# Kainmueller-Lab/PatchPerPix

Hardware: AMD Instinct MI355X
Metric: Mvoxels/sec assembled (vote_instances) (higher is better)
Workload: dtype f16 in, f32 accumulate

## Files before the change

### include/ppp_mi355x.h

```cpp
#ifndef PPP_MI355X_H
#define PPP_MI355X_H

#include <stddef.h>
#include <stdint.h>

#ifdef __cplusplus
extern "C" {
#endif

#define PPP_ABI_VERSION 5

enum ppp_error {
    PPP_OK = 0,
    PPP_ERR_INVALID_ARG = -1,
    PPP_ERR_NO_DEVICE = -2,
    PPP_ERR_HIP = -3,
    PPP_ERR_UNSUPPORTED = -4,
    PPP_ERR_WORKSPACE = -5
};

enum ppp_dtype { PPP_F32 = 0, PPP_F16 = 1, PPP_BF16 = 2 };

enum ppp_bg_rule { PPP_BG_INV_TH = 0, PPP_BG_HALF_TH = 1, PPP_BG_LESS_THAN_TH = 2 };
enum ppp_value_rule { PPP_VAL_COUNT = 0, PPP_VAL_PROB_PRODUCT = 1, PPP_VAL_NORM_PROB_PRODUCT = 2 };
// ... 50 lines not shown

int64_t ppp_consensus_sparse_workspace_bytes(const ppp_params *p, const ppp_box *part);
int ppp_consensus_sparse(const void *d_pred, int pred_dtype, const uint8_t *d_overlap, float *d_cons,
                         float *d_count, const ppp_params *p, const ppp_box *part, int open_rows, void *d_work,
                         int mode, void *stream);
void ppp_consensus_last_items(int64_t *total, int64_t *active, int *took_lists);

int ppp_rank_patches(const void *d_pred, int pred_dtype, const float *d_cons,
                     const uint8_t *d_overlap, float *d_score, const ppp_box *score_box,
                     const ppp_params *p, void *stream);

int64_t ppp_rank_workspace_bytes(const ppp_box *score_box, const ppp_params *p);
int ppp_rank_patches_vm(const void *d_pred, int pred_dtype, const float *d_cons_vm,
                        const uint8_t *d_overlap, float *d_score, const ppp_box *score_box,
                        void *d_work, const ppp_params *p, void *stream);

int ppp_patch_graph(const void *d_pred, int pred_dtype, const float *d_cons,
                    const uint32_t *d_pairs, const uint32_t *d_order, uint64_t n_pairs,
                    float *d_aff, const ppp_params *p, void *stream);

int32_t ppp_patch_graph_by_patch_chunk(const ppp_params *p);
int32_t ppp_patch_graph_by_patch_chunk_small(const ppp_params *p);
int ppp_patch_graph_by_patch_chunked(const void *d_pred, int pred_dtype, const float *d_cons_vm,
                                     const uint32_t *d_pairs, const uint32_t *d_order,
                                     const int64_t *d_group_start, const int64_t *d_chunk_offsets,
                                     int32_t n_groups, int64_t n_blocks, int32_t chunk, float *d_aff,
                                     const ppp_params *p, void *stream);
int64_t ppp_patch_graph_lcg_words(int32_t dz, int32_t dy, int32_t dx, const ppp_params *p);
int ppp_patch_graph_lcg(const void *d_pred, int pred_dtype, const uint32_t *d_pairs,
                        const uint32_t *d_order, const int64_t *d_lcg_pos, int64_t n_lcg,
// ... 291 lines not shown
```

### patchperpix_amd/backend.py

```python
import ctypes
import os

import numpy as np

from . import build as _build

F32, F16, BF16 = 0, 1, 2
BG_INV_TH, BG_HALF_TH, BG_LESS_THAN_TH = 0, 1, 2
VAL_COUNT, VAL_PROB_PRODUCT, VAL_NORM_PROB_PRODUCT = 0, 1, 2
CONS_COMPACT, CONS_REFERENCE, CONS_VOXEL_MAJOR = 0, 1, 2
ABI_VERSION = 5
NONE_KEY = 0xFFFFFFFF
NONE_KEY64 = 1 << 62
PAIR_KEY_FAR = 0x7FFFFFFFFFFFFFFF


class Box(ctypes.Structure):
    _fields_ = [(n, ctypes.c_int32) for n in ("z0", "y0", "x0", "z1", "y1", "x1")]

    def shape(self):
        return (self.z1 - self.z0, self.y1 - self.y0, self.x1 - self.x0)


class Params(ctypes.Structure):
# ... 66 lines not shown
                                          ctypes.c_void_p, ctypes.POINTER(Params), ctypes.POINTER(Box),
                                          ctypes.c_void_p]),
    "ppp_consensus_sparse_workspace_bytes": (ctypes.c_int64, [ctypes.POINTER(Params), ctypes.POINTER(Box)]),
    "ppp_consensus_sparse": (ctypes.c_int, [ctypes.c_void_p, ctypes.c_int, ctypes.c_void_p, ctypes.c_void_p,
                                            ctypes.c_void_p, ctypes.POINTER(Params), ctypes.POINTER(Box),
                                            ctypes.c_int, ctypes.c_void_p, ctypes.c_int, ctypes.c_void_p]),
    "ppp_consensus_last_items": (None, [ctypes.POINTER(ctypes.c_int64), ctypes.POINTER(ctypes.c_int64),
                                        ctypes.POINTER(ctypes.c_int)]),
    "ppp_cons_planes_to_rows": (ctypes.c_int, [ctypes.c_void_p, ctypes.POINTER(Box), ctypes.c_void_p,
                                               ctypes.POINTER(Params), ctypes.c_void_p]),
    "ppp_rank_patches": (ctypes.c_int, [ctypes.c_void_p, ctypes.c_int, ctypes.c_void_p,
                                        ctypes.c_void_p, ctypes.c_void_p,
                                        ctypes.POINTER(Box), ctypes.POINTER(Params),
                                        ctypes.c_void_p]),
    "ppp_rank_workspace_bytes": (ctypes.c_int64, [ctypes.POINTER(Box), ctypes.POINTER(Params)]),
    "ppp_rank_patches_vm": (ctypes.c_int, [ctypes.c_void_p, ctypes.c_int, ctypes.c_void_p,
                                           ctypes.c_void_p, ctypes.c_void_p, ctypes.POINTER(Box),
                                           ctypes.c_void_p, ctypes.POINTER(Params), ctypes.c_void_p]),
    "ppp_patch_graph": (ctypes.c_int, [ctypes.c_void_p, ctypes.c_int, ctypes.c_void_p,
                                       ctypes.c_void_p, ctypes.c_void_p, ctypes.c_uint64,
                                       ctypes.c_void_p, ctypes.POINTER(Params),
                                       ctypes.c_void_p]),
    "ppp_patch_graph_by_patch": (ctypes.c_int, [ctypes.c_void_p, ctypes.c_int, ctypes.c_void_p,
                                                ctypes.c_void_p, ctypes.c_void_p, ctypes.c_void_p,
                                                ctypes.c_void_p, ctypes.c_int32, ctypes.c_int64,
                                                ctypes.c_void_p, ctypes.POINTER(Params),
                                                ctypes.c_void_p]),
    "ppp_patch_graph_by_patch_chunk_small": (ctypes.c_int32, [ctypes.POINTER(Params)]),
    "ppp_patch_graph_by_patch_chunked": (ctypes.c_int, [ctypes.c_void_p, ctypes.c_int, ctypes.c_void_p,
                                                        ctypes.c_void_p, ctypes.c_void_p, ctypes.c_void_p,
# ... 681 lines not shown
        lo3 = [max(sb[a] - rad[a], (cb.z0, cb.y0, cb.x0)[a]) for a in range(3)]
        hi3 = [min(sb[3 + a] + rad[a], (cb.z1, cb.y1, cb.x1)[a]) for a in range(3)]
        note_add("s2_base_voxels", int(np.prod([max(0, h - l) for l, h in zip(lo3, hi3)])))
        with _timed("rank_patches"):
            check(lib().ppp_rank_patches_vm(_dev_ptr(pred), pred_dtype_code(pred), _dev_ptr(cons),
                                            _dev_ptr(overlap), _dev_ptr(out), box, _dev_ptr(work),
                                            ctypes.byref(P), _stream()))
        return out
    with _timed("rank_patches"):
        check(lib().ppp_rank_patches(_dev_ptr(pred), pred_dtype_code(pred), _dev_ptr(cons),
                                     _dev_ptr(overlap), _dev_ptr(out), box, ctypes.byref(P),
                                     _stream()))
    return out


def rank_vm_available(P):
    if os.environ.get("PPP_RANK", "vm") != "vm":
        return False
    Pv = P.copy()
    Pv.cons_layout = CONS_VOXEL_MAJOR
    Pv.cons_box = Box(0, 0, 0, P.Z, P.Y, P.X)
    if P.ring_z and P.ring_z < P.Z:
        Pv.cons_box = Box(0, 0, 0, P.ring_z, P.Y, P.X)
        sb = Box(0, 0, 0, max(1, P.ring_z - P.pz // 2), P.Y, P.X)
        return int(lib().ppp_rank_workspace_bytes(ctypes.byref(sb), ctypes.byref(Pv))) > 0
    return int(lib().ppp_rank_workspace_bytes(None, ctypes.byref(Pv))) > 0


def pair_order(pairs, P):
    torch = _torch()
# ... 1163 lines not shown
```

### patchperpix_amd/csrc/ppp_api.hip

```cpp
#include <cmath>
#include <cstdarg>
#include <cstdio>
#include <cstring>

#include "ppp_kernels.hpp"

namespace {

thread_local char g_err[512] = "";

int fail(int code, const char *fmt, ...) {
    va_list ap;
    va_start(ap, fmt);
    vsnprintf(g_err, sizeof(g_err), fmt, ap);
    va_end(ap);
    return code;
}

int hip_fail(hipError_t e, const char *what) {
    return fail(PPP_ERR_HIP, "%s: %s", what, hipGetErrorString(e));
}

float round_down_f32(double t) {
    float f = (float)t;
// ... 283 lines not shown
    if (!ppp::cons_box_covers(G, *sb))
        return fail(PPP_ERR_INVALID_ARG, "cons_box does not cover score_box grown by the patch radius");
    return PPP_OK;
}

int64_t ppp_rank_workspace_bytes(const ppp_box *score_box, const ppp_params *p) {
    ppp::Geo G;
    if (make_geo(p, &G) != PPP_OK) return -1;
    if (!ppp::rank_vm_supported(G)) return 0;
    if (G.ring && !ppp::rank_wg_supported(G)) return 0;
    ppp_box sb;
    if (rank_box(score_box, p, G, &sb) != PPP_OK) return -1;
    return (int64_t)ppp::rank_vm_workspace_bytes(sb, G);
}

#ifdef PPP_RW_STAMPS
extern "C" int64_t ppp_rank_wg_stamps_offset(const ppp_box *score_box, const ppp_params *p) {
    ppp::Geo G;
    ppp_box sb;
    if (make_geo(p, &G) != PPP_OK || !ppp::rank_wg_supported(G) || rank_box(score_box, p, G, &sb) != PPP_OK) return -1;
    return (int64_t)ppp::rank_wg_stamps_offset(sb, G);
}
#endif

int ppp_rank_patches_vm(const void *d_pred, int pred_dtype, const float *d_cons_vm,
                        const uint8_t *d_overlap, float *d_score, const ppp_box *score_box,
                        void *d_work, const ppp_params *p, void *stream) {
    ppp::Geo G;
    PPP_TRY(make_geo(p, &G));
    PPP_TRY(check_dtype(pred_dtype));
// ... 1259 lines not shown
```

### patchperpix_amd/csrc/ppp_kernels.hpp

```cpp
#pragma once
#include <stdlib.h>
#include <string.h>
#include "ppp_common.hpp"

namespace ppp {

int env_epoch();
void env_reload();
struct EnvSwitch {
    const char *name;
    int seen = -1;
    bool is_set = false;
    char val[32] = {0};
    explicit EnvSwitch(const char *n) : name(n) {}
    const char *get() {
        if (seen != env_epoch()) {
            const char *e = getenv(name);
            is_set = e != nullptr;
            if (e) { strncpy(val, e, sizeof(val) - 1); val[sizeof(val) - 1] = 0; }
            seen = env_epoch();
        }
        return is_set ? val : nullptr;
    }
};
// ... 27 lines not shown
hipError_t launch_consensus_part(const void *pred, int dtype, const uint8_t *ov, float *cons, const Geo &G,
                                 hipStream_t s);
bool consensus_v4_supported(const Geo &G);
hipError_t launch_consensus_v4(const void *pred, int dtype, const uint8_t *ov, float *cons,
                               float *cnt, const Geo &G, hipStream_t s);
hipError_t launch_rank(const void *pred, int dtype, const float *cons, const uint8_t *ov,
                       float *score, const ppp_box &sb, const Geo &G, hipStream_t s);
hipError_t launch_rank_v2(const void *pred, int dtype, const float *cons, const uint8_t *ov,
                          float *score, const ppp_box &sb, const Geo &G, hipStream_t s);
bool rank_vm_supported(const Geo &G);
size_t rank_vm_workspace_bytes(const ppp_box &sb, const Geo &G);
hipError_t launch_rank_vm(const void *pred, int dtype, const float *S, const uint8_t *ov, float *score,
                          const ppp_box &sb, void *work, const Geo &G, hipStream_t s);
bool rank_wg_supported(const Geo &G);
size_t rank_wg_workspace_bytes(const ppp_box &sb, const Geo &G);
#ifdef PPP_RW_STAMPS
size_t rank_wg_stamps_offset(const ppp_box &sb, const Geo &G);
#endif
hipError_t launch_rank_wg(const void *pred, int dtype, const float *S, const uint8_t *ov, float *score,
                          const ppp_box &sb, void *work, const Geo &G, hipStream_t s);
hipError_t launch_patch_graph(const void *pred, int dtype, const float *cons,
                              const uint32_t *pairs, const uint32_t *order, uint64_t n,
                              float *aff, const Geo &G, hipStream_t s);
int patch_graph_pa_chunk(const Geo &G, bool small = false);
hipError_t launch_patch_graph_pa(const void *pred, int dtype, const float *S, const uint32_t *rows,
                                 const uint32_t *order, const long long *group_start,
                                 const long long *chunk_offsets, int n_groups, long long n_blocks,
                                 int chunk, float *aff, const long long *drop_off,
                                 const unsigned long long *drops, const long long *bits_centres, int n_bits,
                                 const uint32_t *bits, const Geo &G, hipStream_t s);
// ... 171 lines not shown
```

### patchperpix_amd/csrc/ppp_rank_wg.hip

```cpp
#include <stdlib.h>
#include <string.h>

#include <type_traits>

#include "ppp_kernels.hpp"

namespace ppp {

#ifndef PPP_RW_MINWAVES
#define PPP_RW_MINWAVES(PX) 4
#endif
#ifndef PPP_RW_ZRUNS
#define PPP_RW_ZRUNS(PX) ((PX) == 9)
#endif
#ifndef PPP_RW_BANKDEAL
#define PPP_RW_BANKDEAL(PX) ((PX) == 7)
#endif
static constexpr int RW_PAD = 8;
#ifndef PPP_RW_WAVES
#define PPP_RW_WAVES 4
#endif
#ifndef PPP_RW_REVREADS
#define PPP_RW_REVREADS 1
#endif
// ... 35 lines not shown
};
template <int END>
struct StaticFor<END, END> {
    template <class F>
    static __device__ __forceinline__ void run(F &&) {}
};

__host__ __device__ __forceinline__ uint32_t interleave16(uint32_t p, uint32_t n) {
    uint32_t out = 0;
#pragma unroll
    for (int j = 0; j < 4; ++j)
        out |= (((p >> (4 * j)) & 0xFu) | (((n >> (4 * j)) & 0xFu) << 4)) << (8 * j);
    return out;
}

template <typename T>
__global__ void __launch_bounds__(256)
    rank_masks_il_kernel(const T *__restrict__ pred, const uint8_t *__restrict__ ov, const ppp_box sb,
                         uint32_t *__restrict__ M, uint32_t *__restrict__ info,
                         float *__restrict__ score, const int *__restrict__ any_e, const Geo G) {
    if (any_e && *any_e == 0) return;
    const int sX = sb.x1 - sb.x0, sY = sb.y1 - sb.y0, sZ = sb.z1 - sb.z0;
    const long long sbV = (long long)sX * sY * sZ;
    const long long t = (long long)blockIdx.x * blockDim.x + threadIdx.x;
    if (t >= sbV) return;
    const int cx = sb.x0 + (int)(t % sX), cy = sb.y0 + (int)((t / sX) % sY), cz = sb.z0 + (int)(t / ((long long)sX * sY));
    const long long lc = vox(G, cz, cy, cx);
    const T *mid = pred + (long long)G.mid * G.V;
    uint32_t inf = 0;
    if (!interior(G, cz, cy, cx)) {
        score[lc] = G.norm_rank ? -1.0f : -9999999.0f;
    } else if (!(ldf(mid, lc) > G.th_gt)) {
        score[lc] = 0.0f;
    } else {
        const int words16 = (G.C + 15) / 16;
        const long long q0 = rw_mask_quad0(t / sX, (int)(t % sX), sX, rw_mask_words(G.C) / 4);
        unsigned nP = 0, nV = 0;
        int r = 0;
        for (int w = 0; w < words16; ++w) {
            uint32_t p = 0, n = 0;
            for (int b = 0; b < 16 && r < G.C; ++b, ++r) {
                const int z = cz + r / (G.py * G.px) - G.rz, y = cy + (r / G.px) % G.py - G.ry,
                          x = cx + r % G.px - G.rx;
                const long long lz = vox(G, z, y, x);
                const bool valid = ldf(mid, lz) > G.th_gt && (!G.use_overlap || ov[lz] == 0);
                const float val = ldf(pred, (long long)r * G.V + lc);
                if (valid) ++nV;
                if (valid && val > G.th_gt) p |= 1u << b;
                if (valid && val < G.bg_lt) n |= 1u << b;
            }
            M[(q0 + (long long)(w >> 2) * RW_QSTRIDE) * 4 + (w & 3)] = interleave16(p, n);
            nP += __popc(p);
        }
        for (int w = words16; w < rw_mask_words(G.C); ++w) M[(q0 + (long long)(w >> 2) * RW_QSTRIDE) * 4 + (w & 3)] = 0u;
        const unsigned fg_cnt = nP ? nP * (nV - 1u) - nP * (nP - 1u) / 2u : 0u;
        inf = 0x80000000u | fg_cnt;
        if (nP == 0) score[lc] = 0.0f;
    }
    info[t] = inf;
}

static constexpr int rw_p1_words(int C) { return (((C + 31) / 32) + 3) & ~3; }
template <typename T>
__global__ void __launch_bounds__(256)
    rank_masks_p1_kernel(const T *__restrict__ pred, const uint8_t *__restrict__ ov, const ppp_box sb,
                         uint32_t *__restrict__ M, uint32_t *__restrict__ info, int *__restrict__ any_e,
                         float *__restrict__ score, const Geo G) {
    const int sX = sb.x1 - sb.x0, sY = sb.y1 - sb.y0, sZ = sb.z1 - sb.z0;
    const long long sbV = (long long)sX * sY * sZ;
    const long long t = (long long)blockIdx.x * blockDim.x + threadIdx.x;
    if (t >= sbV) return;
    const int cx = sb.x0 + (int)(t % sX), cy = sb.y0 + (int)((t / sX) % sY), cz = sb.z0 + (int)(t / ((long long)sX * sY));
    const long long lc = vox(G, cz, cy, cx);
    const T *mid = pred + (long long)G.mid * G.V;
    uint32_t inf = 0;
    if (!interior(G, cz, cy, cx)) {
        score[lc] = G.norm_rank ? -1.0f : -9999999.0f;
    } else if (!(ldf(mid, lc) > G.th_gt)) {
        score[lc] = 0.0f;
    } else {
        const int words = (G.C + 31) / 32, wp = rw_p1_words(G.C);
        unsigned nP = 0, nV = 0;
        bool e = false;
        int r = 0;
        for (int w = 0; w < words; ++w) {
            uint32_t p = 0;
            for (int b = 0; b < 32 && r < G.C; ++b, ++r) {
                const int z = cz + r / (G.py * G.px) - G.rz, y = cy + (r / G.px) % G.py - G.ry,
                          x = cx + r % G.px - G.rx;
                const long long lz = vox(G, z, y, x);
                const bool valid = ldf(mid, lz) > G.th_gt && (!G.use_overlap || ov[lz] == 0);
                const float val = ldf(pred, (long long)r * G.V + lc);
                const bool isp = val > G.th_gt;
                if (valid) ++nV;
                if (valid && isp) ++nP;
                if (valid && !isp && !(val < G.bg_lt)) e = true;
                if (isp) p |= 1u << b;
            }
            M[t * (long long)wp + w] = p;
// ... 59 lines not shown
        }
    }
    for (int o = 32; o > 0; o >>= 1) { c += __shfl_xor(c, o); w += __shfl_xor(w, o); }
    __shared__ int part[2][4];
    if ((threadIdx.x & 63) == 0) { part[0][threadIdx.x >> 6] = c; part[1][threadIdx.x >> 6] = w; }
    __syncthreads();
    if (threadIdx.x == 0) {
        const int cs = part[0][0] + part[0][1] + part[0][2] + part[0][3];
        const int ws = part[1][0] + part[1][1] + part[1][2] + part[1][3];
        weight[bid] = by_centres ? cs : (cs ? ws : 0);
    }
}
static constexpr int32_t RW_HALF_LO = 1 << 28, RW_HALF_HI = 2 << 28, RW_TILE_MASK = (1 << 28) - 1;
__global__ void __launch_bounds__(256)
    rank_tile_order_kernel(const int32_t *__restrict__ weight, const int n_tiles, const int per_xcd, const int splits,
                           int32_t *__restrict__ order) {
    __shared__ int32_t w[RW_ORDER_MAX / 8 + 8];
    __shared__ int32_t key[RW_ORDER_MAX / 8 + 8];
    const int lo = blockIdx.x * per_xcd, hi = min(lo + per_xcd, n_tiles), n = max(hi - lo, 0);
    const int slot0 = blockIdx.x * (per_xcd + splits);
    for (int i = threadIdx.x; i < n; i += blockDim.x) w[i] = weight[lo + i];
    for (int t = threadIdx.x; t < per_xcd + splits; t += blockDim.x) order[slot0 + t] = -1;
    __syncthreads();
    for (int i = threadIdx.x; i < n; i += blockDim.x) {
        const int wi = w[i];
        int before = 0, with_work = 0;
        for (int j = 0; j < n; ++j) {
            before += (w[j] > wi || (w[j] == wi && j < i)) ? 1 : 0;
            with_work += w[j] > 0 ? 1 : 0;
        }
        key[i] = (wi > 0 && before >= with_work - splits) ? (((wi + 1) >> 1) | (1 << 30)) : wi;
    }
    __syncthreads();
    for (int i = threadIdx.x; i < n; i += blockDim.x) {
        const int ki = key[i] & ~(1 << 30);
        int before = 0;
        for (int j = 0; j < n; ++j) {
// ... 35 lines not shown
        }
    n_over[r] = k > H ? min(k - H, MAXOVER) : 0;
    __syncthreads();
    if (r == 0) {
        int f = 0;
        for (int rr = 0; rr < 32; ++rr)
            for (int o = 0; o < n_over[rr]; ++o) {
                while (f < 32 * H && slot[f] != 0) ++f;
                if (f < 32 * H) slot[f] = over[rr][o];
            }
    }
    __syncthreads();
    for (int i = r; i < SLOTS; i += 32) T[(size_t)cls * SLOTS + i] = slot[i];
}

template <int PZ, int PY, int PX, int TZ, int TY, int TX, bool P1>
__global__ void __launch_bounds__(64 * RW_WAVES, PPP_RW_MINWAVES(PX))
    rank_wg_kernel(const float *__restrict__ S, const uint32_t *__restrict__ M,
                   const uint32_t *__restrict__ info, const uint8_t *__restrict__ valid,
                   float *__restrict__ score, const ppp_box sb, const Geo G, const int tiles_y,
                   const int tiles_x, const int n_tiles, const int *__restrict__ any_e,
                   const int32_t *__restrict__ order, const int y_major, const uint16_t *__restrict__ dealT
#ifdef PPP_RW_STAMPS
                   , uint32_t *__restrict__ stamps
#endif
                   ) {
    if (any_e && (*any_e != 0) == P1) return;
#ifdef PPP_RW_STAMPS
    const unsigned long long t_start = wall_clock64();
#endif
    constexpr int C = PZ * PY * PX, W16 = (C + 15) / 16, RZ = PZ / 2, RY = PY / 2, RX = PX / 2;
    constexpr int W16P = P1 ? rw_p1_words(C) : rw_mask_words(C);
    constexpr int NMW = P1 ? (C + 31) / 32 : W16;
    constexpr int WZ = 2 * PZ - 1, WY = 2 * PY - 1, WX = 2 * PX - 1, W = WZ * WY * WX, LC = (W - 1) / 2;
    constexpr int NTHR = 64 * RW_WAVES;
    constexpr int NST = (W + NTHR - 1) / NTHR;
    constexpr int NT = TZ * TY * TX;
// ... 9 lines not shown
    __shared__ uint32_t uvalid_bits[(UB + 63) / 64 * 2];
    __shared__ int any_act;
    const int tid = threadIdx.x, lane = tid & 63;
    const int wave = __builtin_amdgcn_readfirstlane(tid >> 6);
    const int sX = sb.x1 - sb.x0, sY = sb.y1 - sb.y0, sZ = sb.z1 - sb.z0;
    const long long sbV = (long long)sX * sY * sZ;
    const int n_blocks = gridDim.x;
    const int per_xcd = (n_blocks + 7) / 8;
    const int slot = (blockIdx.x & 7) * per_xcd + (blockIdx.x >> 3);
    const int rec = order ? order[slot] : slot;
    if (rec < 0) return;
    const int bid = rec & RW_TILE_MASK, half_hi = (rec & RW_HALF_HI) ? 1 : 0, halved = (rec & (RW_HALF_LO | RW_HALF_HI)) ? 1 : 0;
    if (bid >= n_tiles) return;
    int tx_i, ty_i, tz_i;
    rw_tile_decode(bid, n_tiles, tiles_y, tiles_x, y_major, tz_i, ty_i, tx_i);
    const int c0z = sb.z0 + tz_i * TZ, c0y = sb.y0 + ty_i * TY + half_hi * (TY / 2), c0x = sb.x0 + tx_i * TX;
    const int tz = min(TZ, sb.z1 - c0z), ty = min(halved ? TY / 2 : TY, sb.y1 - c0y), tx = min(TX, sb.x1 - c0x);
    if (tz <= 0 || ty <= 0 || tx <= 0) return;

    auto sb_index = [&](int lz, int ly, int lx) -> long long {
        return ((long long)(c0z + lz - sb.z0) * sY + (c0y + ly - sb.y0)) * sX + (c0x + lx - sb.x0);
    };
    for (int e = tid; e < 256; e += NTHR) {
        uint32_t h[4];
#pragma unroll
        for (int i = 0; i < 4; ++i) h[i] = ((e >> i) & 1) ? 0x2800u : (((e >> (4 + i)) & 1) ? 0xA800u : 0u);
        coefT[e] = make_uint2(h[0] | (h[1] << 16), h[2] | (h[3] << 16));
    }
    if (tid == 0) any_act = 0;
    __syncthreads();
    static_assert(NT % 64 == 0, "tile size must be a multiple of the wave size");
    for (int cl = tid; cl < NT; cl += NTHR) {
        const int lx = cl % TX, ly = (cl / TX) % TY, lz = cl / (TX * TY);
        uint32_t v = 0;
        if (lz < tz && ly < ty && lx < tx) v = info[sb_index(lz, ly, lx)];
        const unsigned long long m = __ballot((v >> 31) != 0);
        if (lane == 0) {
            act_bits[cl >> 5] = (uint32_t)m; act_bits[(cl >> 5) + 1] = (uint32_t)(m >> 32);
            if (m) any_act = 1;
        }
        accs[cl] = 0.0f;
    }
    __syncthreads();
    if (!any_act) return;

    const long long rsY = G.bX, rsZ = (long long)G.bX * G.bY;
    const int uz0 = max(c0z - RZ, G.bz0), uz1 = min(c0z + tz - 1 + RZ, G.bz0 + G.bZ - 1);
// ... 241 lines not shown
                }
            });
            if (active) accs[cl] = acc;
        }
        __syncthreads();
        if (uk_next < nu) {
#pragma unroll
            for (int i = 0; i < NST; ++i) {
                const int e = tid + i * NTHR;
                if (e < W) rowbuf[RW_PAD + img(e)] = st[i] * 32.0f;
            }
        }
        __syncthreads();
        uk = uk_next;
    }
    for (int cl = tid; cl < NT; cl += NTHR) {
        const int lx = cl % TX, ly = (cl / TX) % TY, lz = cl / (TX * TY);
        if (lz < tz && ly < ty && lx < tx && ((act_bits[cl >> 5] >> (cl & 31)) & 1u)) {
            const unsigned fg_cnt = info[sb_index(lz, ly, lx)] & 0x7FFFFFFFu;
            const float acc = accs[cl];
            score[vox(G, c0z + lz, c0y + ly, c0x + lx)] = G.norm_rank ? acc / (float)(fg_cnt > 1u ? fg_cnt : 1u) : acc;
        }
    }
#ifdef PPP_RW_STAMPS
    if (tid == 0 && stamps && blockIdx.x < RW_ORDER_MAX / 4) {
        const unsigned long long t_end = wall_clock64();
        unsigned hw_id;
        asm volatile("s_getreg_b32 %0, hwreg(HW_REG_HW_ID)" : "=s"(hw_id));
        unsigned xcc_id;
        asm volatile("s_getreg_b32 %0, hwreg(HW_REG_XCC_ID)" : "=s"(xcc_id));
        stamps[4 * blockIdx.x + 0] = (uint32_t)t_start;
// ... 33 lines not shown
}
size_t rank_wg_workspace_bytes(const ppp_box &sb, const Geo &G) { Carver c(nullptr); rank_wg_layout(c, sb, G); return c.used; }
#ifdef PPP_RW_STAMPS
size_t rank_wg_stamps_offset(const ppp_box &sb, const Geo &G) {
    char base;
    Carver c(&base);
    return (size_t)((char *)rank_wg_layout(c, sb, G).weight - &base);
}
#endif

static int rw_choose_splits(int tiles_per_xcd, int slots_per_xcd) {
    if (slots_per_xcd <= 0 || tiles_per_xcd <= slots_per_xcd) return 0;
    const int rem = tiles_per_xcd % slots_per_xcd;
    return 2 * rem <= slots_per_xcd ? rem : 0;
}
template <int P>
static int rw_resident_per_cu() {
    static thread_local int memo = 0;
    if (memo == 0) {
        int nb = 0;
        if (hipOccupancyMaxActiveBlocksPerMultiprocessor(&nb, rank_wg_kernel<P, P, P, 8, 16, 16, false>, 64 * RW_WAVES, 0) != hipSuccess || nb < 1)
            nb = PPP_RW_MINWAVES(P);
        memo = nb;
    }
    return memo;
}
static int rw_cus_per_xcd() {
    static thread_local int memo = 0;
    if (memo == 0) {
        int dev = 0, cus = 0;
        if (hipGetDevice(&dev) != hipSuccess || hipDeviceGetAttribute(&cus, hipDeviceAttributeMultiprocessorCount, dev) != hipSuccess || cus < 8)
            cus = 256;
        memo = cus / 8;
    }
    return memo;
}

template <typename T>
static hipError_t launch_rwg(const T *pred, const float *S, const uint8_t *ov, float *score,
                             const ppp_box &sb, void *work, const Geo &G, hipStream_t s) {
    const int sX = sb.x1 - sb.x0, sY = sb.y1 - sb.y0, sZ = sb.z1 - sb.z0;
    const size_t sbV = (size_t)sX * sY * sZ;
    Carver carver(work);
    auto [M, info, valid, any_e, weight, order, dealT] = rank_wg_layout(carver, sb, G);
    if (!cons_box_covers(G, sb)) return hipErrorInvalidValue;
    PPP_GRID_CHECK((G.V + 255) / 256, 256);
    PPP_GRID_CHECK((sbV + 255) / 256, 256);
    rank_valid2_kernel<T><<<dim3((unsigned)((G.V + 255) / 256)), dim3(256), 0, s>>>(pred, ov, valid, G);
    static EnvSwitch p1_sw("PPP_RANK_P1");
    const bool p1 = G.bg_lt >= G.th_gt && p1_sw.get() && p1_sw.get()[0] == '1';
    note_rank_kernel(p1 ? "rank_wg_kernel<p1>" : "rank_wg_kernel");
    if (p1) {
        hipError_t em = hipMemsetAsync(any_e, 0, 4, s);
        if (em != hipSuccess) return em;
        rank_masks_p1_kernel<T><<<dim3((unsigned)((sbV + 255) / 256)), dim3(256), 0, s>>>(pred, ov, sb, M, info, any_e,
                                                                                          score, G);
    }
    const long long big_tiles = (long long)((sZ + 7) / 8) * ((sY + 15) / 16) * ((sX + 15) / 16);
    bool big = big_tiles >= 4 * 256;
    static EnvSwitch tile_sw("PPP_RANK_WG_TILE");
    if (const char *e = tile_sw.get()) big = strcmp(e, "8x16x16") == 0 ? true : (strcmp(e, "8x8x16") == 0 ? false : big);
    if (G.px == 9 && PPP_RW_ZRUNS(9) && !tile_sw.get()) big = false;
    bool tall = tile_sw.get() && strcmp(tile_sw.get(), "16x8x16") == 0;
    if (G.rank_tile && !tile_sw.get()) { big = G.rank_tile == 2; tall = G.rank_tile == 3; }
    const int TZ = tall ? 16 : 8, TY = tall ? 8 : (big ? 16 : 8), TX = 16;
    const int tiles_z = (sZ + TZ - 1) / TZ, tiles_y = (sY + TY - 1) / TY, tiles_x = (sX + TX - 1) / TX;
    const long long n_tiles = (long long)tiles_z * tiles_y * tiles_x;
    const int per_xcd = (int)((n_tiles + 7) / 8);
    static EnvSwitch order_sw("PPP_RANK_ORDER");
    if (n_tiles > RW_ORDER_MAX || (order_sw.get() && order_sw.get()[0] == '0')) order = nullptr;
    static EnvSwitch split_sw("PPP_RANK_WG_SPLIT");
    int splits = 0;
    if (order) {
        if (split_sw.get() && split_sw.get()[0] >= '0' && split_sw.get()[0] <= '9') splits = atoi(split_sw.get());
        else if (big && !tall && !tile_sw.get() && !G.rank_tile)
            splits = rw_choose_splits(per_xcd, rw_cus_per_xcd() * (G.px == 5 ? rw_resident_per_cu<5>() : (G.px == 7 ? rw_resident_per_cu<7>() : rw_resident_per_cu<9>())));
        splits = splits < per_xcd ? splits : per_xcd;
        if (8LL * (per_xcd + splits) > RW_ORDER_MAX) splits = RW_ORDER_MAX / 8 - per_xcd;
    }
    const long long n_blocks = 8LL * (per_xcd + splits);
    PPP_GRID_CHECK(n_blocks, 64 * RW_WAVES);
    const bool by_centres = order_sw.get() && order_sw.get()[0] == 'c';
    static EnvSwitch major_sw("PPP_RANK_TILE_MAJOR");
    const int y_major = (major_sw.get() && major_sw.get()[0] == 'z') ? 0 : 1;
    static EnvSwitch dyn_sw("PPP_RANK_WG_DYNLDS");
    const unsigned dyn_lds = dyn_sw.get() ? (unsigned)atoi(dyn_sw.get()) : 0u;
#ifdef PPP_RW_STAMPS
#define PPP_RW_STAMP_ARG , (uint32_t *)weight
#else
#define PPP_RW_STAMP_ARG
#endif
#define PPP_RW_LAUNCH1(A_, D_, E_, F_, P1_)                                                                 \
    rank_wg_kernel<A_, A_, A_, D_, E_, F_, P1_><<<dim3((unsigned)n_blocks), dim3(64 * RW_WAVES), dyn_lds, s>>>( \
        S, M, info, valid, score, sb, G, tiles_y, tiles_x, (int)n_tiles, p1 ? any_e : nullptr, order, y_major, dealT PPP_RW_STAMP_ARG)
#define PPP_RW_LAUNCH(A_, D_, E_, F_)                                                                       \
    do {                                                                                                    \
        if (p1 && pass == 0) PPP_RW_LAUNCH1(A_, D_, E_, F_, true);                                          \
        else PPP_RW_LAUNCH1(A_, D_, E_, F_, false);                                                         \
    } while (0)
#define PPP_RW_CASE(P)                                                                                      \
    case P:                                                                                                 \
        if (tall) PPP_RW_LAUNCH(P, 16, 8, 16);                                                              \
        else if (big) PPP_RW_LAUNCH(P, 8, 16, 16);                                                          \
        else PPP_RW_LAUNCH(P, 8, 8, 16);                                                                    \
        break;
    if (PPP_RW_BANKDEAL(7) && G.px == 7)
        rank_deal_table_kernel<7><<<dim3(7 * 7 * 7), dim3(32), 0, s>>>(dealT, 2 * 7 - 1, (2 * 7 - 1) * (2 * 7 - 1));
    for (int pass = p1 ? 0 : 1; pass < 2; ++pass) {
        if (pass == 1)
            rank_masks_il_kernel<T><<<dim3((unsigned)((sbV + 255) / 256)), dim3(256), 0, s>>>(pred, ov, sb, M, info, score,
                                                                                              p1 ? any_e : nullptr, G);
        if (order && pass == (p1 ? 0 : 1)) {
            rank_tile_weight_kernel<<<dim3((unsigned)n_tiles), dim3(256), 0, s>>>(info, valid, sb, TZ, TY, TX, tiles_y, tiles_x,
                                                                                  by_centres ? 1 : 0, y_major, weight, G);
            rank_tile_order_kernel<<<dim3(8), dim3(256), 0, s>>>(weight, (int)n_tiles, per_xcd, splits, order);
        }
#ifdef PPP_RW_STAMPS
        (void)hipMemsetAsync(weight, 0, (size_t)RW_ORDER_MAX * 4, s);
#endif
        switch (G.px) {
            PPP_RW_CASE(5)
            PPP_RW_CASE(7)
            PPP_RW_CASE(9)
        default:
            return hipErrorNotSupported;
        }
    }
#undef PPP_RW_LAUNCH
#undef PPP_RW_LAUNCH1
#undef PPP_RW_STAMP_ARG
#undef PPP_RW_CASE
    return hipGetLastError();
}

hipError_t launch_rank_wg(const void *pred, int dtype, const float *S, const uint8_t *ov, float *score,
                          const ppp_box &sb, void *work, const Geo &G, hipStream_t s) {
    if (!rank_wg_supported(G)) return hipErrorNotSupported;
    return with_pred_type(dtype, [&](auto tag) {
        using T = PPP_PRED_T(tag);
        return launch_rwg<T>((const T *)pred, S, ov, score, sb, work, G, s);
    });
}

}
```

Measured before the change: 15.24.

## Plan rank_wg tiling to fit one wave, balance XCDs by weight, specialize mask kernels

Moves the rank workgroup tile planning into a reusable planner. For px=7 it can pick a variable-depth 16x16x16 tile (tz_step 9..16) so that all tiles fit in one resident wave per XCD instead of spilling into a partial second wave. The tile order kernel can also split tiles across XCDs by cumulative weight rather than by count. Separately, the mask precompute kernels get a compile-time patch-size path that reads the valid mask per row instead of per element. This adds template instantiations and planner complexity, and the fit path only applies to px=7.

```diff
diff --git a/include/ppp_mi355x.h b/include/ppp_mi355x.h
--- a/include/ppp_mi355x.h
+++ b/include/ppp_mi355x.h
@@ -88,6 +88,8 @@
 int ppp_rank_patches_vm(const void *d_pred, int pred_dtype, const float *d_cons_vm,
                         const uint8_t *d_overlap, float *d_score, const ppp_box *score_box,
                         void *d_work, const ppp_params *p, void *stream);
+int ppp_rank_wg_plan(const ppp_box *score_box, const ppp_params *p, int resident_per_cu, int cus_per_xcd,
+                     int32_t plan[8]);
 
 int ppp_patch_graph(const void *d_pred, int pred_dtype, const float *d_cons,
                     const uint32_t *d_pairs, const uint32_t *d_order, uint64_t n_pairs,
diff --git a/patchperpix_amd/backend.py b/patchperpix_amd/backend.py
--- a/patchperpix_amd/backend.py
+++ b/patchperpix_amd/backend.py
@@ -104,6 +104,8 @@
                                         ctypes.POINTER(Box), ctypes.POINTER(Params),
                                         ctypes.c_void_p]),
     "ppp_rank_workspace_bytes": (ctypes.c_int64, [ctypes.POINTER(Box), ctypes.POINTER(Params)]),
+    "ppp_rank_wg_plan": (ctypes.c_int, [ctypes.POINTER(Box), ctypes.POINTER(Params), ctypes.c_int, ctypes.c_int,
+                                        ctypes.POINTER(ctypes.c_int32)]),
     "ppp_rank_patches_vm": (ctypes.c_int, [ctypes.c_void_p, ctypes.c_int, ctypes.c_void_p,
                                            ctypes.c_void_p, ctypes.c_void_p, ctypes.POINTER(Box),
                                            ctypes.c_void_p, ctypes.POINTER(Params), ctypes.c_void_p]),
@@ -815,6 +817,14 @@
     return out
 
 
+def rank_wg_plan(P, score_box=None, resident_per_cu=0, cus_per_xcd=0):
+    box = None if score_box is None else ctypes.byref(Box(*[int(v) for v in score_box]))
+    out = (ctypes.c_int32 * 8)()
+    check(lib().ppp_rank_wg_plan(box, ctypes.byref(P), int(resident_per_cu), int(cus_per_xcd), out))
+    return dict(tile=(out[0], out[1], out[2]), tz_step=out[3], tiles=out[4], splits=out[5], slots=out[6],
+                ranges="weight" if out[7] else "count")
+
+
 def rank_vm_available(P):
     if os.environ.get("PPP_RANK", "vm") != "vm":
         return False
diff --git a/patchperpix_amd/csrc/ppp_api.hip b/patchperpix_amd/csrc/ppp_api.hip
--- a/patchperpix_amd/csrc/ppp_api.hip
+++ b/patchperpix_amd/csrc/ppp_api.hip
@@ -321,6 +321,19 @@
     return (int64_t)ppp::rank_vm_workspace_bytes(sb, G);
 }
 
+int ppp_rank_wg_plan(const ppp_box *score_box, const ppp_params *p, int resident_per_cu, int cus_per_xcd, int32_t *plan) {
+    ppp::Geo G;
+    PPP_TRY(make_geo(p, &G));
+    if (!plan) return fail(PPP_ERR_INVALID_ARG, "NULL pointer argument");
+    if (!ppp::rank_wg_supported(G))
+        return fail(PPP_ERR_UNSUPPORTED, "ppp_rank_wg_plan: the workgroup-per-tile kernel does not serve these parameters");
+    ppp_box sb;
+    PPP_TRY(rank_box(score_box, p, G, &sb));
+    if (resident_per_cu <= 0 || cus_per_xcd <= 0) PPP_TRY(need_device());
+    ppp::rank_wg_plan(sb, G, resident_per_cu, cus_per_xcd, plan);
+    return PPP_OK;
+}
+
 #ifdef PPP_RW_STAMPS
 extern "C" int64_t ppp_rank_wg_stamps_offset(const ppp_box *score_box, const ppp_params *p) {
     ppp::Geo G;
diff --git a/patchperpix_amd/csrc/ppp_kernels.hpp b/patchperpix_amd/csrc/ppp_kernels.hpp
--- a/patchperpix_amd/csrc/ppp_kernels.hpp
+++ b/patchperpix_amd/csrc/ppp_kernels.hpp
@@ -65,6 +65,7 @@
                           const ppp_box &sb, void *work, const Geo &G, hipStream_t s);
 bool rank_wg_supported(const Geo &G);
 size_t rank_wg_workspace_bytes(const ppp_box &sb, const Geo &G);
+void rank_wg_plan(const ppp_box &sb, const Geo &G, int resident_per_cu, int cus_per_xcd, int32_t out[8]);
 #ifdef PPP_RW_STAMPS
 size_t rank_wg_stamps_offset(const ppp_box &sb, const Geo &G);
 #endif
diff --git a/patchperpix_amd/csrc/ppp_rank_wg.hip b/patchperpix_amd/csrc/ppp_rank_wg.hip
--- a/patchperpix_amd/csrc/ppp_rank_wg.hip
+++ b/patchperpix_amd/csrc/ppp_rank_wg.hip
@@ -73,10 +73,10 @@
     return out;
 }
 
-template <typename T>
+template <typename T, int P>
 __global__ void __launch_bounds__(256)
-    rank_masks_il_kernel(const T *__restrict__ pred, const uint8_t *__restrict__ ov, const ppp_box sb,
-                         uint32_t *__restrict__ M, uint32_t *__restrict__ info,
+    rank_masks_il_kernel(const T *__restrict__ pred, const uint8_t *__restrict__ ov, const uint8_t *__restrict__ valid_v,
+                         const ppp_box sb, uint32_t *__restrict__ M, uint32_t *__restrict__ info,
                          float *__restrict__ score, const int *__restrict__ any_e, const Geo G) {
     if (any_e && *any_e == 0) return;
     const int sX = sb.x1 - sb.x0, sY = sb.y1 - sb.y0, sZ = sb.z1 - sb.z0;
@@ -96,6 +96,29 @@
         const long long q0 = rw_mask_quad0(t / sX, (int)(t % sX), sX, rw_mask_words(G.C) / 4);
         unsigned nP = 0, nV = 0;
         int r = 0;
+        if constexpr (P != 0) {
+            constexpr int R = P / 2, C = P * P * P;
+            uint32_t p = 0, n = 0;
+            for (int dz = 0; dz < P; ++dz)
+                for (int dy = 0; dy < P; ++dy) {
+                    const uint8_t *vrow = valid_v + vox(G, cz + dz - R, cy + dy - R, cx - R);
+#pragma unroll
+                    for (int dx = 0; dx < P; ++dx, ++r) {
+                        const bool valid = vrow[dx] != 0;
+                        const float val = ldf(pred, (long long)r * G.V + lc);
+                        const int b = r & 15;
+                        if (valid) ++nV;
+                        if (valid && val > G.th_gt) p |= 1u << b;
+                        if (valid && val < G.bg_lt) n |= 1u << b;
+                        if (b == 15 || r == C - 1) {
+                            const int w = r >> 4;
+                            M[(q0 + (long long)(w >> 2) * RW_QSTRIDE) * 4 + (w & 3)] = interleave16(p, n);
+                            nP += __popc(p);
+                            p = n = 0;
+                        }
+                    }
+                }
+        } else
         for (int w = 0; w < words16; ++w) {
             uint32_t p = 0, n = 0;
             for (int b = 0; b < 16 && r < G.C; ++b, ++r) {
@@ -120,10 +143,10 @@
 }
 
 static constexpr int rw_p1_words(int C) { return (((C + 31) / 32) + 3) & ~3; }
-template <typename T>
+template <typename T, int P>
 __global__ void __launch_bounds__(256)
-    rank_masks_p1_kernel(const T *__restrict__ pred, const uint8_t *__restrict__ ov, const ppp_box sb,
-                         uint32_t *__restrict__ M, uint32_t *__restrict__ info, int *__restrict__ any_e,
+    rank_masks_p1_kernel(const T *__restrict__ pred, const uint8_t *__restrict__ ov, const uint8_t *__restrict__ valid_v,
+                         const ppp_box sb, uint32_t *__restrict__ M, uint32_t *__restrict__ info, int *__restrict__ any_e,
                          float *__restrict__ score, const Geo G) {
     const int sX = sb.x1 - sb.x0, sY = sb.y1 - sb.y0, sZ = sb.z1 - sb.z0;
     const long long sbV = (long long)sX * sY * sZ;
@@ -142,6 +165,26 @@
         unsigned nP = 0, nV = 0;
         bool e = false;
         int r = 0;
+        if constexpr (P != 0) {
+            constexpr int R = P / 2, C = P * P * P;
+            uint32_t p = 0;
+            for (int dz = 0; dz < P; ++dz)
+                for (int dy = 0; dy < P; ++dy) {
+                    const uint8_t *vrow = valid_v + vox(G, cz + dz - R, cy + dy - R, cx - R);
+#pragma unroll
+                    for (int dx = 0; dx < P; ++dx, ++r) {
+                        const bool valid = vrow[dx] != 0;
+                        const float val = ldf(pred, (long long)r * G.V + lc);
+                        const bool isp = val > G.th_gt;
+                        const int b = r & 31;
+                        if (valid) ++nV;
+                        if (valid && isp) ++nP;
+                        if (valid && !isp && !(val < G.bg_lt)) e = true;
+                        if (isp) p |= 1u << b;
+                        if (b == 31 || r == C - 1) { M[t * (long long)wp + (r >> 5)] = p; p = 0; }
+                    }
+                }
+        } else
         for (int w = 0; w < words; ++w) {
             uint32_t p = 0;
             for (int b = 0; b < 32 && r < G.C; ++b, ++r) {
@@ -231,13 +274,45 @@
 static constexpr int32_t RW_HALF_LO = 1 << 28, RW_HALF_HI = 2 << 28, RW_TILE_MASK = (1 << 28) - 1;
 __global__ void __launch_bounds__(256)
     rank_tile_order_kernel(const int32_t *__restrict__ weight, const int n_tiles, const int per_xcd, const int splits,
-                           int32_t *__restrict__ order) {
+                           const int slots, const int by_weight, int32_t *__restrict__ order) {
     __shared__ int32_t w[RW_ORDER_MAX / 8 + 8];
     __shared__ int32_t key[RW_ORDER_MAX / 8 + 8];
-    const int lo = blockIdx.x * per_xcd, hi = min(lo + per_xcd, n_tiles), n = max(hi - lo, 0);
-    const int slot0 = blockIdx.x * (per_xcd + splits);
+    __shared__ int part_sum[256];
+    __shared__ int cut[9];
+    int lo = blockIdx.x * per_xcd, hi = min(lo + per_xcd, n_tiles);
+    if (by_weight) {
+        const int ch = (n_tiles + 255) / 256;
+        int ps = 0;
+        for (int i = threadIdx.x * ch; i < min((threadIdx.x + 1) * ch, n_tiles); ++i) ps += weight[i];
+        part_sum[threadIdx.x] = ps;
+        __syncthreads();
+        if (threadIdx.x < 9) {
+            long long total = 0;
+            for (int c = 0; c < 256; ++c) total += part_sum[c];
+            int at = threadIdx.x == 8 ? n_tiles : 0;
+            if (threadIdx.x > 0 && threadIdx.x < 8) {
+                const long long want = (total * threadIdx.x + 7) / 8;
+                long long run = 0;
+                int c = 0;
+                while (c < 256 && run + part_sum[c] < want) run += part_sum[c++];
+                at = min(c * ch, n_tiles);
+                while (at < n_tiles && run < want) run += weight[at++];
+            }
+            cut[threadIdx.x] = at;
+        }
+        __syncthreads();
+        if (threadIdx.x == 0) {
+            const int cap = min(slots - splits, RW_ORDER_MAX / 8);
+            for (int k = 1; k < 8; ++k)
+                cut[k] = min(max(max(cut[k], cut[k - 1]), n_tiles - (8 - k) * cap), cut[k - 1] + cap);
+        }
+        __syncthreads();
+        lo = cut[blockIdx.x]; hi = cut[blockIdx.x + 1];
+    }
+    const int n = max(hi - lo, 0);
+    const int slot0 = blockIdx.x * slots;
     for (int i = threadIdx.x; i < n; i += blockDim.x) w[i] = weight[lo + i];
-    for (int t = threadIdx.x; t < per_xcd + splits; t += blockDim.x) order[slot0 + t] = -1;
+    for (int t = threadIdx.x; t < slots; t += blockDim.x) order[slot0 + t] = -1;
     __syncthreads();
     for (int i = threadIdx.x; i < n; i += blockDim.x) {
         const int wi = w[i];
@@ -303,13 +378,14 @@
     for (int i = r; i < SLOTS; i += 32) T[(size_t)cls * SLOTS + i] = slot[i];
 }
 
-template <int PZ, int PY, int PX, int TZ, int TY, int TX, bool P1>
+template <int PZ, int PY, int PX, int TZ, int TY, int TX, bool P1, bool DZ = false>
 __global__ void __launch_bounds__(64 * RW_WAVES, PPP_RW_MINWAVES(PX))
     rank_wg_kernel(const float *__restrict__ S, const uint32_t *__restrict__ M,
                    const uint32_t *__restrict__ info, const uint8_t *__restrict__ valid,
                    float *__restrict__ score, const ppp_box sb, const Geo G, const int tiles_y,
                    const int tiles_x, const int n_tiles, const int *__restrict__ any_e,
-                   const int32_t *__restrict__ order, const int y_major, const uint16_t *__restrict__ dealT
+                   const int32_t *__restrict__ order, const int y_major, const uint16_t *__restrict__ dealT,
+                   const int tz_step
 #ifdef PPP_RW_STAMPS
                    , uint32_t *__restrict__ stamps
 #endif
@@ -349,8 +425,9 @@
     if (bid >= n_tiles) return;
     int tx_i, ty_i, tz_i;
     rw_tile_decode(bid, n_tiles, tiles_y, tiles_x, y_major, tz_i, ty_i, tx_i);
-    const int c0z = sb.z0 + tz_i * TZ, c0y = sb.y0 + ty_i * TY + half_hi * (TY / 2), c0x = sb.x0 + tx_i * TX;
-    const int tz = min(TZ, sb.z1 - c0z), ty = min(halved ? TY / 2 : TY, sb.y1 - c0y), tx = min(TX, sb.x1 - c0x);
+    const int tzs = DZ ? min(tz_step, TZ) : TZ;
+    const int c0z = sb.z0 + tz_i * tzs, c0y = sb.y0 + ty_i * TY + half_hi * (TY / 2), c0x = sb.x0 + tx_i * TX;
+    const int tz = min(tzs, sb.z1 - c0z), ty = min(halved ? TY / 2 : TY, sb.y1 - c0y), tx = min(TX, sb.x1 - c0x);
     if (tz <= 0 || ty <= 0 || tx <= 0) return;
 
     auto sb_index = [&](int lz, int ly, int lx) -> long long {
@@ -364,8 +441,9 @@
     }
     if (tid == 0) any_act = 0;
     __syncthreads();
-    static_assert(NT % 64 == 0, "tile size must be a multiple of the wave size");
-    for (int cl = tid; cl < NT; cl += NTHR) {
+    static_assert(NT % 64 == 0 && (TY * TX) % 64 == 0, "tile size must be a multiple of the wave size");
+    const int nt_used = DZ ? tz * TY * TX : NT;
+    for (int cl = tid; cl < nt_used; cl += NTHR) {
         const int lx = cl % TX, ly = (cl / TX) % TY, lz = cl / (TX * TY);
         uint32_t v = 0;
         if (lz < tz && ly < ty && lx < tx) v = info[sb_index(lz, ly, lx)];
@@ -637,7 +715,7 @@
         __syncthreads();
         uk = uk_next;
     }
-    for (int cl = tid; cl < NT; cl += NTHR) {
+    for (int cl = tid; cl < nt_used; cl += NTHR) {
         const int lx = cl % TX, ly = (cl / TX) % TY, lz = cl / (TX * TY);
         if (lz < tz && ly < ty && lx < tx && ((act_bits[cl >> 5] >> (cl & 31)) & 1u)) {
             const unsigned fg_cnt = info[sb_index(lz, ly, lx)] & 0x7FFFFFFFu;
@@ -701,13 +779,15 @@
     const int rem = tiles_per_xcd % slots_per_xcd;
     return 2 * rem <= slots_per_xcd ? rem : 0;
 }
-template <int P>
+template <int P, bool FIT>
 static int rw_resident_per_cu() {
     static thread_local int memo = 0;
     if (memo == 0) {
         int nb = 0;
-        if (hipOccupancyMaxActiveBlocksPerMultiprocessor(&nb, rank_wg_kernel<P, P, P, 8, 16, 16, false>, 64 * RW_WAVES, 0) != hipSuccess || nb < 1)
-            nb = PPP_RW_MINWAVES(P);
+        hipError_t e;
+        if constexpr (FIT) e = hipOccupancyMaxActiveBlocksPerMultiprocessor(&nb, rank_wg_kernel<P, P, P, 16, 16, 16, false, true>, 64 * RW_WAVES, 0);
+        else e = hipOccupancyMaxActiveBlocksPerMultiprocessor(&nb, rank_wg_kernel<P, P, P, 8, 16, 16, false>, 64 * RW_WAVES, 0);
+        if (e != hipSuccess || nb < 1) nb = PPP_RW_MINWAVES(P);
         memo = nb;
     }
     return memo;
@@ -721,6 +801,80 @@
         memo = cus / 8;
     }
     return memo;
+}
+
+struct RwPlan {
+    int TZ, TY, TX;
+    int tz_step;
+    bool fit;
+    int tiles_z, tiles_y, tiles_x;
+    long long n_tiles;
+    int per_xcd, splits, slots;
+    bool ordered, by_weight;
+};
+static int rw_env_int(EnvSwitch &sw, int none) {
+    const char *e = sw.get();
+    return (e && e[0] >= '0' && e[0] <= '9') ? atoi(e) : none;
+}
+static RwPlan rw_plan(const ppp_box &sb, const Geo &G, int resident, int resident_fit, int cus_per_xcd) {
+    const int sX = sb.x1 - sb.x0, sY = sb.y1 - sb.y0, sZ = sb.z1 - sb.z0;
+    RwPlan p{};
+    const long long big_tiles = (long long)((sZ + 7) / 8) * ((sY + 15) / 16) * ((sX + 15) / 16);
+    bool big = big_tiles >= 4 * 256;
+    static EnvSwitch tile_sw("PPP_RANK_WG_TILE");
+    if (const char *e = tile_sw.get()) big = strcmp(e, "8x16x16") == 0 ? true : (strcmp(e, "8x8x16") == 0 ? false : big);
+    if (G.px == 9 && PPP_RW_ZRUNS(9) && !tile_sw.get()) big = false;
+    bool tall = tile_sw.get() && strcmp(tile_sw.get(), "16x8x16") == 0;
+    if (G.rank_tile && !tile_sw.get()) { big = G.rank_tile == 2; tall = G.rank_tile == 3; }
+    const bool by_rule = big && !tall && !tile_sw.get() && !G.rank_tile;
+    p.TZ = tall ? 16 : 8; p.TY = tall ? 8 : (big ? 16 : 8); p.TX = 16;
+    p.tz_step = p.TZ;
+    static EnvSwitch order_sw("PPP_RANK_ORDER");
+    static EnvSwitch split_sw("PPP_RANK_WG_SPLIT");
+    static EnvSwitch tz_sw("PPP_RANK_WG_TZ");
+    static EnvSwitch xcd_sw("PPP_RANK_WG_XCD");
+    const int split_env = rw_env_int(split_sw, -1);
+    const int tz_env = G.px == 7 ? rw_env_int(tz_sw, 0) : 0;
+    const int slots_res = resident * cus_per_xcd, slots_fit = resident_fit * cus_per_xcd;
+    auto tiles_of = [&](int t, int ty) { return (long long)((sZ + t - 1) / t) * ((sY + ty - 1) / ty) * ((sX + 15) / 16); };
+    if (tz_env > 0) {
+        p.fit = true; p.TZ = 16; p.TY = 16; p.TX = 16;
+        p.tz_step = tz_env < 16 ? tz_env : 16;
+    } else if (by_rule && G.px == 7 && split_env < 0) {
+        const long long per0 = (tiles_of(8, 16) + 7) / 8;
+        if (slots_res > 0 && per0 > slots_res && per0 < 2LL * slots_res)
+            for (int t = 9; t <= 16; ++t)
+                if ((tiles_of(t, 16) + 7) / 8 <= slots_fit) { p.fit = true; p.TZ = 16; p.tz_step = t; break; }
+    }
+    p.tiles_z = (sZ + p.tz_step - 1) / p.tz_step; p.tiles_y = (sY + p.TY - 1) / p.TY; p.tiles_x = (sX + p.TX - 1) / p.TX;
+    p.n_tiles = (long long)p.tiles_z * p.tiles_y * p.tiles_x;
+    p.per_xcd = (int)((p.n_tiles + 7) / 8);
+    p.ordered = !(p.n_tiles > RW_ORDER_MAX || (order_sw.get() && order_sw.get()[0] == '0'));
+    p.slots = p.per_xcd;
+    if (p.ordered) {
+        if (split_env >= 0) p.splits = split_env;
+        else if (by_rule && !p.fit) p.splits = rw_choose_splits(p.per_xcd, slots_res);
+        p.splits = p.splits < p.per_xcd ? p.splits : p.per_xcd;
+        if (8LL * (p.per_xcd + p.splits) > RW_ORDER_MAX) p.splits = RW_ORDER_MAX / 8 - p.per_xcd;
+        p.by_weight = p.fit && tz_env == 0;
+        if (const char *e = xcd_sw.get()) p.by_weight = strcmp(e, "weight") == 0 ? true : (strcmp(e, "count") == 0 ? false : p.by_weight);
+        p.slots = p.per_xcd + p.splits;
+        if (p.by_weight) {
+            p.slots += (p.per_xcd + 3) / 4;
+            if (8LL * p.slots > RW_ORDER_MAX) p.slots = RW_ORDER_MAX / 8;
+        }
+    }
+    return p;
+}
+static RwPlan rw_plan_device(const ppp_box &sb, const Geo &G) {
+    const int res = G.px == 5 ? rw_resident_per_cu<5, false>() : (G.px == 7 ? rw_resident_per_cu<7, false>() : rw_resident_per_cu<9, false>());
+    return rw_plan(sb, G, res, G.px == 7 ? rw_resident_per_cu<7, true>() : res, rw_cus_per_xcd());
+}
+void rank_wg_plan(const ppp_box &sb, const Geo &G, int resident_per_cu, int cus_per_xcd, int32_t out[8]) {
+    const RwPlan p = (resident_per_cu > 0 && cus_per_xcd > 0) ? rw_plan(sb, G, resident_per_cu, resident_per_cu, cus_per_xcd)
+                                                              : rw_plan_device(sb, G);
+    out[0] = p.TZ; out[1] = p.TY; out[2] = p.TX; out[3] = p.tz_step;
+    out[4] = (int32_t)p.n_tiles; out[5] = p.splits; out[6] = p.slots; out[7] = p.by_weight ? 1 : 0;
 }
 
 template <typename T>
@@ -737,36 +891,29 @@
     static EnvSwitch p1_sw("PPP_RANK_P1");
     const bool p1 = G.bg_lt >= G.th_gt && p1_sw.get() && p1_sw.get()[0] == '1';
     note_rank_kernel(p1 ? "rank_wg_kernel<p1>" : "rank_wg_kernel");
+    static EnvSwitch cube_sw("PPP_RANK_PRE_CUBE");
+    const int pre_p = (cube_sw.get() && cube_sw.get()[0] == '0') ? 0 : G.px;
+    const dim3 pre_grid((unsigned)((sbV + 255) / 256));
+#define PPP_RW_PRE(KERNEL_, ...)                                                                            \
+    do {                                                                                                    \
+        if (pre_p == 5) KERNEL_<T, 5><<<pre_grid, dim3(256), 0, s>>>(__VA_ARGS__);                          \
+        else if (pre_p == 7) KERNEL_<T, 7><<<pre_grid, dim3(256), 0, s>>>(__VA_ARGS__);                     \
+        else if (pre_p == 9) KERNEL_<T, 9><<<pre_grid, dim3(256), 0, s>>>(__VA_ARGS__);                     \
+        else KERNEL_<T, 0><<<pre_grid, dim3(256), 0, s>>>(__VA_ARGS__);                                     \
+    } while (0)
     if (p1) {
         hipError_t em = hipMemsetAsync(any_e, 0, 4, s);
         if (em != hipSuccess) return em;
-        rank_masks_p1_kernel<T><<<dim3((unsigned)((sbV + 255) / 256)), dim3(256), 0, s>>>(pred, ov, sb, M, info, any_e,
-                                                                                          score, G);
-    }
-    const long long big_tiles = (long long)((sZ + 7) / 8) * ((sY + 15) / 16) * ((sX + 15) / 16);
-    bool big = big_tiles >= 4 * 256;
-    static EnvSwitch tile_sw("PPP_RANK_WG_TILE");
-    if (const char *e = tile_sw.get()) big = strcmp(e, "8x16x16") == 0 ? true : (strcmp(e, "8x8x16") == 0 ? false : big);
-    if (G.px == 9 && PPP_RW_ZRUNS(9) && !tile_sw.get()) big = false;
-    bool tall = tile_sw.get() && strcmp(tile_sw.get(), "16x8x16") == 0;
-    if (G.rank_tile && !tile_sw.get()) { big = G.rank_tile == 2; tall = G.rank_tile == 3; }
-    const int TZ = tall ? 16 : 8, TY = tall ? 8 : (big ? 16 : 8), TX = 16;
-    const int tiles_z = (sZ + TZ - 1) / TZ, tiles_y = (sY + TY - 1) / TY, tiles_x = (sX + TX - 1) / TX;
-    const long long n_tiles = (long long)tiles_z * tiles_y * tiles_x;
-    const int per_xcd = (int)((n_tiles + 7) / 8);
+        PPP_RW_PRE(rank_masks_p1_kernel, pred, ov, valid, sb, M, info, any_e, score, G);
+    }
+    const RwPlan plan = rw_plan_device(sb, G);
+    const bool tall = plan.TZ == 16 && !plan.fit, big = plan.TY == 16, fit = plan.fit;
+    const int tiles_y = plan.tiles_y, tiles_x = plan.tiles_x, per_xcd = plan.per_xcd, splits = plan.splits, tz_step = plan.tz_step;
+    const long long n_tiles = plan.n_tiles;
+    if (!plan.ordered) order = nullptr;
+    const long long n_blocks = 8LL * plan.slots;
+    PPP_GRID_CHECK(n_blocks, 64 * RW_WAVES);
     static EnvSwitch order_sw("PPP_RANK_ORDER");
-    if (n_tiles > RW_ORDER_MAX || (order_sw.get() && order_sw.get()[0] == '0')) order = nullptr;
-    static EnvSwitch split_sw("PPP_RANK_WG_SPLIT");
-    int splits = 0;
-    if (order) {
-        if (split_sw.get() && split_sw.get()[0] >= '0' && split_sw.get()[0] <= '9') splits = atoi(split_sw.get());
-        else if (big && !tall && !tile_sw.get() && !G.rank_tile)
-            splits = rw_choose_splits(per_xcd, rw_cus_per_xcd() * (G.px == 5 ? rw_resident_per_cu<5>() : (G.px == 7 ? rw_resident_per_cu<7>() : rw_resident_per_cu<9>())));
-        splits = splits < per_xcd ? splits : per_xcd;
-        if (8LL * (per_xcd + splits) > RW_ORDER_MAX) splits = RW_ORDER_MAX / 8 - per_xcd;
-    }
-    const long long n_blocks = 8LL * (per_xcd + splits);
-    PPP_GRID_CHECK(n_blocks, 64 * RW_WAVES);
     const bool by_centres = order_sw.get() && order_sw.get()[0] == 'c';
     static EnvSwitch major_sw("PPP_RANK_TILE_MAJOR");
     const int y_major = (major_sw.get() && major_sw.get()[0] == 'z') ? 0 : 1;
@@ -777,34 +924,37 @@
 #else
 #define PPP_RW_STAMP_ARG
 #endif
-#define PPP_RW_LAUNCH1(A_, D_, E_, F_, P1_)                                                                 \
-    rank_wg_kernel<A_, A_, A_, D_, E_, F_, P1_><<<dim3((unsigned)n_blocks), dim3(64 * RW_WAVES), dyn_lds, s>>>( \
-        S, M, info, valid, score, sb, G, tiles_y, tiles_x, (int)n_tiles, p1 ? any_e : nullptr, order, y_major, dealT PPP_RW_STAMP_ARG)
-#define PPP_RW_LAUNCH(A_, D_, E_, F_)                                                                       \
+#define PPP_RW_LAUNCH1(A_, D_, E_, F_, P1_, DZ_)                                                            \
+    rank_wg_kernel<A_, A_, A_, D_, E_, F_, P1_, DZ_><<<dim3((unsigned)n_blocks), dim3(64 * RW_WAVES), dyn_lds, s>>>( \
+        S, M, info, valid, score, sb, G, tiles_y, tiles_x, (int)n_tiles, p1 ? any_e : nullptr, order, y_major, dealT, tz_step PPP_RW_STAMP_ARG)
+#define PPP_RW_LAUNCH(A_, D_, E_, F_, DZ_)                                                                  \
     do {                                                                                                    \
-        if (p1 && pass == 0) PPP_RW_LAUNCH1(A_, D_, E_, F_, true);                                          \
-        else PPP_RW_LAUNCH1(A_, D_, E_, F_, false);                                                         \
+        if (p1 && pass == 0) PPP_RW_LAUNCH1(A_, D_, E_, F_, true, DZ_);                                     \
+        else PPP_RW_LAUNCH1(A_, D_, E_, F_, false, DZ_);                                                    \
     } while (0)
 #define PPP_RW_CASE(P)                                                                                      \
     case P:                                                                                                 \
-        if (tall) PPP_RW_LAUNCH(P, 16, 8, 16);                                                              \
-        else if (big) PPP_RW_LAUNCH(P, 8, 16, 16);                                                          \
-        else PPP_RW_LAUNCH(P, 8, 8, 16);                                                                    \
+        if (tall) PPP_RW_LAUNCH(P, 16, 8, 16, false);                                                       \
+        else if (big) PPP_RW_LAUNCH(P, 8, 16, 16, false);                                                   \
+        else PPP_RW_LAUNCH(P, 8, 8, 16, false);                                                             \
         break;
     if (PPP_RW_BANKDEAL(7) && G.px == 7)
         rank_deal_table_kernel<7><<<dim3(7 * 7 * 7), dim3(32), 0, s>>>(dealT, 2 * 7 - 1, (2 * 7 - 1) * (2 * 7 - 1));
     for (int pass = p1 ? 0 : 1; pass < 2; ++pass) {
-        if (pass == 1)
-            rank_masks_il_kernel<T><<<dim3((unsigned)((sbV + 255) / 256)), dim3(256), 0, s>>>(pred, ov, sb, M, info, score,
-                                                                                              p1 ? any_e : nullptr, G);
+        if (pass == 1) PPP_RW_PRE(rank_masks_il_kernel, pred, ov, valid, sb, M, info, score, p1 ? any_e : nullptr, G);
         if (order && pass == (p1 ? 0 : 1)) {
-            rank_tile_weight_kernel<<<dim3((unsigned)n_tiles), dim3(256), 0, s>>>(info, valid, sb, TZ, TY, TX, tiles_y, tiles_x,
+            rank_tile_weight_kernel<<<dim3((unsigned)n_tiles), dim3(256), 0, s>>>(info, valid, sb, tz_step, plan.TY, plan.TX, tiles_y, tiles_x,
                                                                                   by_centres ? 1 : 0, y_major, weight, G);
-            rank_tile_order_kernel<<<dim3(8), dim3(256), 0, s>>>(weight, (int)n_tiles, per_xcd, splits, order);
+            rank_tile_order_kernel<<<dim3(8), dim3(256), 0, s>>>(weight, (int)n_tiles, per_xcd, splits, plan.slots,
+                                                                 plan.by_weight ? 1 : 0, order);
         }
 #ifdef PPP_RW_STAMPS
         (void)hipMemsetAsync(weight, 0, (size_t)RW_ORDER_MAX * 4, s);
 #endif
+        if (fit) {
+            if (G.px != 7) return hipErrorNotSupported;
+            PPP_RW_LAUNCH(7, 16, 16, 16, true);
+        } else
         switch (G.px) {
             PPP_RW_CASE(5)
             PPP_RW_CASE(7)
@@ -817,6 +967,7 @@
 #undef PPP_RW_LAUNCH1
 #undef PPP_RW_STAMP_ARG
 #undef PPP_RW_CASE
+#undef PPP_RW_PRE
     return hipGetLastError();
 }
 
```

New measurement: 15.89, median of 6. 1.04x the previous value.
